# andrenarchy/krypy

Hardware: AMD Instinct MI355X
Metric: GMRES iterations/sec + SpMV HBM GB/s, n=10^7 5-pt Laplacian fp64 (higher is better)
Workload: dtype f64; 1 GPU; GMRES(100) restart cycles, 2-D 5-pt Laplacian 4000x2500 CSR (N=10000000, nnz=49987000), b=rng(0) normal, x0=0, tol=1e-8 (BASELINE.json configs[1]); n=10000000, ortho=mgs, restart=100, parallelism=1 GPU, ranks=1

## Files before the change

### krypy_amd/csrc/chain.h

```cpp
#pragma once
#include <type_traits>
#include "kernels.h"

namespace kh {

constexpr int CH_BS = 512;
constexpr int CH_GMAX = 512;

struct ChainArgs {
    int64_t n2;
    int64_t chunk2;
    const double* V;
    const double* B;
    int64_t ld;
    int64_t col0;
    int ncol;
    int sweeps;
    const double* w_in;
    const double* dg;
    double* vnext;
    double* pnext;
    double* hdev;
    int64_t hnext;
    unsigned long long* gran;
// ... 525 lines not shown
            int64_t c = row + a.offs.off[d];
            c = c < 0 ? 0 : (c > last ? last : c);
            xv[d] = xk[c];
        }
        double sx = 0.0, sy = 0.0;
#pragma unroll
        for (int d = 0; d < FND; ++d) {
            const double px = av[d].x * xv[d].x - av[d].y * xv[d].y;
            const double py = av[d].x * xv[d].y + av[d].y * xv[d].x;
            const bool on = (av[d].x != 0.0) || (av[d].y != 0.0);
            sx = on ? sx + px : sx;
            sy = on ? sy + py : sy;
        }
        put(r, sx, sy);
        if ((r & 1) == 1) asm volatile("" : "+v"(fb) : : "memory");
    }
}

template <int R2, int FND, int RIF, bool MASK, class Put>
__device__ __forceinline__ void chain_apply_banded_form(const ChainArgs& a, int64_t first, Put&& put) {
    const double* __restrict__ xk = a.xk;
    const int64_t last = a.n_last;
    int64_t fb = first;
#pragma unroll
    for (int r = 0; r < R2; ++r) {
        const int64_t i2 = fb + (int64_t)r * CH_BS;
        const int64_t row = 2 * i2;
        double2 av[FND];
        double x0[FND], x1[FND];
        const unsigned m = MASK ? dia_mask_load(a.dmask, i2) : 0u;
#pragma unroll
        for (int d = 0; d < FND; ++d) {
            const int64_t off = a.offs.off[d];
            av[d] = dia_slot<MASK>(a.dia, a.dia_ld, d, i2, m, MASK ? a.offs.cst[d] : 0.0);
            int64_t c0 = row + off, c1 = row + 1 + off;
            c0 = c0 < 0 ? 0 : (c0 > last ? last : c0);
            c1 = c1 < 0 ? 0 : (c1 > last ? last : c1);
            x0[d] = xk[c0];
            x1[d] = xk[c1];
        }
        double s0 = 0.0, s1 = 0.0;
#pragma unroll
        for (int d = 0; d < FND; ++d) {
            const double p0 = av[d].x * x0[d], p1 = av[d].y * x1[d];
            s0 = (av[d].x != 0.0) ? s0 + p0 : s0;
            s1 = (av[d].y != 0.0) ? s1 + p1 : s1;
        }
        put(r, s0, s1);
        if ((r & RIF) == RIF) asm volatile("" : "+v"(fb) : : "memory");
    }
}

template <int R2, int FND, int RIF = KH_RIF, class Put>
__device__ __forceinline__ void chain_apply_banded(const ChainArgs& a, int64_t first, Put&& put) {
    static_assert(FND <= KH_DIA_CMAX, "the mask form holds up to KH_DIA_CMAX diagonals");
    if (a.dmask != nullptr) chain_apply_banded_form<R2, FND, RIF, true>(a, first, put);
    else chain_apply_banded_form<R2, FND, RIF, false>(a, first, put);
}

template <int R2, bool MASKED, bool CPLX = false, int FND = 0, int WL = 0, bool ONEX = false, bool XR = false>
__global__ __launch_bounds__(CH_BS) void k_mgs_chain(ChainArgs a) {
    static_assert(FND == 0 || !MASKED, "the fused operator exists for the padded kernels");
    static_assert(!XR || (!CPLX && !ONEX), "the cross-rank stage exists for real vectors spread over the chip");
    constexpr int RW = R2 - WL;
    extern __shared__ __attribute__((aligned(16))) double2 wl[];
#define W_GET(r) (((r) < RW) ? w[((r) < RW) ? (r) : 0] : wl[((r) - RW) * CH_BS + tid])
#define W_PUT(r, val)                                   \
    do {                                                \
        if ((r) < RW) w[((r) < RW) ? (r) : 0] = (val);  \
        else wl[((r) - RW) * CH_BS + tid] = (val);      \
    } while (0)
    constexpr int PB = ChainShape<R2>::PB;
    constexpr int NB = ChainShape<R2>::NB;
    __shared__ double smd[4 * (CH_BS / 64)];
    __shared__ unsigned smu[2 * CH_GMAX];
    __shared__ int slead;
    const int tid = threadIdx.x;
    int G = gridDim.x;
    int bid = blockIdx.x;
    GridRole role;
    if constexpr (ONEX) {
        if (!onex_enter(a, &slead, bid, G, role)) return;
    } else {
        role = grid_role(a.xcc_leader, a.epoch0, &slead);
    }
    const int64_t first = (int64_t)bid * a.chunk2 + tid;
    const int64_t left = a.n2 - first;
    const int rem = (int)(left < 0 ? 0 : (left > a.chunk2 ? a.chunk2 : left));
#define CH_OK(r) (!MASKED || (r) * CH_BS < rem)
    double2 w[RW];
    double2 ring[2][PB];
    if constexpr (FND > 0 && CPLX) {
        chain_apply_banded_z<R2, FND>(a, first, [&](int r, double s0, double s1) { W_PUT(r, make_double2(s0, s1)); });
    } else if constexpr (FND > 0) {
        chain_apply_banded<R2, FND>(a, first, [&](int r, double s0, double s1) { W_PUT(r, make_double2(s0, s1)); });
    } else {
        const double2* __restrict__ win2 = reinterpret_cast<const double2*>(a.w_in) + first;
#pragma unroll
        for (int r = 0; r < R2; ++r) {
            const double2 v = win2[(int64_t)r * CH_BS];
            double2 t;
            t.x = CH_OK(r) ? v.x : 0.0;
            t.y = CH_OK(r) ? v.y : 0.0;
            W_PUT(r, t);
            if ((r + 1) % 8 == 0) CH_ISSUE_FENCE();
        }
    }
    if (a.presub) {
        const double hk = (a.h_km1_dev != nullptr) ? a.h_km1_dev[0] : a.h_km1;
        const double2* __restrict__ p2 = reinterpret_cast<const double2*>(a.bprev) + first;
#pragma unroll
        for (int r = 0; r < R2; ++r) {
            const double2 p = p2[(int64_t)r * CH_BS];
            double2 t = W_GET(r);
            t.x = CH_OK(r) ? t.x - hk * p.x : 0.0;
            t.y = CH_OK(r) ? t.y - hk * p.y : 0.0;
            W_PUT(r, t);
            if ((r + 1) % 8 == 0) CH_ISSUE_FENCE();
        }
    }
    unsigned epoch = a.epoch0;
    if (a.debug == 4 && tid == 0) __hip_atomic_store(a.err, 1, __ATOMIC_RELAXED, __HIP_MEMORY_SCOPE_AGENT);
    const int total = a.ncol * a.sweeps;
    {
        const double2* __restrict__ v2 = reinterpret_cast<const double2*>(a.V + a.col0 * a.ld) + first;
#pragma unroll
        for (int i = 0; i < PB; ++i) ring[0][i] = v2[(int64_t)i * CH_BS];
        CH_ISSUE_FENCE();
    }
    for (int t = 0; t < total; ++t) {
        const int64_t j = a.col0 + (t % a.ncol);
        const double2* __restrict__ v2 = reinterpret_cast<const double2*>(a.V + j * a.ld) + first;
        const double2* __restrict__ b2 = reinterpret_cast<const double2*>(a.B + j * a.ld) + first;
        double acc0 = 0.0, acc1 = 0.0;
        if (a.debug != 2)
#pragma unroll
        for (int b = 0; b < NB; ++b) {
            const double2* __restrict__ nx = (b + 1 < NB) ? v2 + (int64_t)(b + 1) * PB * CH_BS : b2;
#pragma unroll
            for (int i = 0; i < PB; ++i)
                ring[(b + 1) & 1][i] = (WL > 0 && b + 1 == NB) ? ld_nt2(nx + (int64_t)i * CH_BS) : nx[(int64_t)i * CH_BS];
            CH_ISSUE_FENCE();
#pragma unroll
            for (int i = 0; i < PB; ++i) {
                double2 v = ring[b & 1][i];
                if (MASKED && !CH_OK(b * PB + i)) v = make_double2(0.0, 0.0);
                const double2 wr = W_GET(b * PB + i);
                if (CPLX) {
                    acc0 = fma(v.x, wr.x, acc0);
                    acc0 = fma(v.y, wr.y, acc0);
                    acc1 = fma(v.x, wr.y, acc1);
                    acc1 = fma(-v.y, wr.x, acc1);
                } else {
                    acc0 = fma(v.x, wr.x, acc0);
                    acc1 = fma(v.y, wr.y, acc1);
                }
            }
        }
        double alpha, alpha_i = 0.0;
        if (CPLX) {
            alpha = acc0;
            alpha_i = acc1;
            if constexpr (ONEX) {
                double pv[2] = {alpha, alpha_i};
                onex_sum<2>(pv, epoch++, a.gran, G, bid, a.err, smd);
                alpha = pv[0];
                alpha_i = pv[1];
            } else {
                grid_sum2(alpha, alpha_i, epoch++, a.gran, G, a.err, smd, smu, role, a.xcc_res);
            }
            if (bid == 0 && tid == 0) {
                a.hdev[2 * j] = (t < a.ncol ? 0.0 : a.hdev[2 * j]) + alpha;
                a.hdev[2 * j + 1] = (t < a.ncol ? 0.0 : a.hdev[2 * j + 1]) + alpha_i;
            }
        } else {
            if constexpr (ONEX) {
                double pv[1] = {acc0 + acc1};
                onex_sum<1>(pv, epoch++, a.gran, G, bid, a.err, smd);
                alpha = pv[0];
            } else {
                const unsigned e_ = epoch++;
                alpha = (a.debug == 1) ? (acc0 + acc1) * 1e-30
                                       : grid_sum<XR>(acc0 + acc1, e_, a.gran, G, a.err, smd, smu, role, a.xcc_res, nullptr, &a.xr,
                                                      a.xr.epoch0 + (e_ - a.epoch0));
            }
            if (bid == 0 && tid == 0) a.hdev[j] = (t < a.ncol ? 0.0 : a.hdev[j]) + alpha;
        }
        if (a.debug == 4) alpha *= 0.5;
        const int64_t jn = a.col0 + ((t + 1) % a.ncol);
        const double2* __restrict__ vn = (t + 1 < total)
            ? reinterpret_cast<const double2*>(a.V + jn * a.ld) + first
            : reinterpret_cast<const double2*>(a.w_in) + first;
        if (a.debug != 2)
#pragma unroll
        for (int b = 0; b < NB; ++b) {
            const double2* __restrict__ nx = (b + 1 < NB) ? b2 + (int64_t)(b + 1) * PB * CH_BS : vn;
#pragma unroll
            for (int i = 0; i < PB; ++i)
                ring[(b + 1) & 1][i] = (WL > 0 && b + 1 < NB) ? ld_nt2(nx + (int64_t)i * CH_BS) : nx[(int64_t)i * CH_BS];
            CH_ISSUE_FENCE();
#pragma unroll
            for (int i = 0; i < PB; ++i) {
                const double2 p = ring[b & 1][i];
                const int r = b * PB + i;
                double2 wr = W_GET(r);
                if (CPLX) {
                    const double tr = alpha * p.x - alpha_i * p.y;
                    const double ti = alpha * p.y + alpha_i * p.x;
                    wr.x = CH_OK(r) ? wr.x - tr : 0.0;
                    wr.y = CH_OK(r) ? wr.y - ti : 0.0;
                } else {
                    wr.x = CH_OK(r) ? wr.x - alpha * p.x : 0.0;
                    wr.y = CH_OK(r) ? wr.y - alpha * p.y : 0.0;
                }
                W_PUT(r, wr);
            }
        }
    }
    double acc = 0.0;
    if (a.dg != nullptr) {
        const double2* __restrict__ d2 = reinterpret_cast<const double2*>(a.dg) + first;
#pragma unroll
        for (int r = 0; r < R2; ++r) {
            const double2 d = d2[(int64_t)r * CH_BS];
            const double2 wr = W_GET(r);
            acc = fma(wr.x, d.x * wr.x, acc);
            acc = fma(wr.y, d.y * wr.y, acc);
            if ((r + 1) % 8 == 0) CH_ISSUE_FENCE();
        }
    } else {
#pragma unroll
        for (int r = 0; r < R2; ++r) {
            const double2 wr = W_GET(r);
            acc = fma(wr.x, wr.x, acc);
            acc = fma(wr.y, wr.y, acc);
        }
    }
    double h2;
    if constexpr (ONEX) {
        double pv[1] = {acc};
        onex_sum<1>(pv, epoch++, a.gran, G, bid, a.err, smd);
        h2 = pv[0];
    } else {
        const unsigned e_ = epoch++;
        h2 = grid_sum<XR>(acc, e_, a.gran, G, a.err, smd, smu, role, a.xcc_res, nullptr, &a.xr, a.xr.epoch0 + (e_ - a.epoch0));
    }
    const double h = sqrt(fabs(h2));
    if (bid == 0 && tid == 0) a.hdev[a.hnext] = h;
    double2* __restrict__ vn2 = reinterpret_cast<double2*>(a.vnext) + first;
    if (a.dg != nullptr) {
        double2* __restrict__ pn2 = reinterpret_cast<double2*>(a.pnext) + first;
        const double2* __restrict__ d2 = reinterpret_cast<const double2*>(a.dg) + first;
#pragma unroll
        for (int r = 0; r < R2; ++r) {
            if (r * CH_BS < rem) {
                const double2 d = d2[(int64_t)r * CH_BS];
                const double2 wr = W_GET(r);
                double2 o, m;
                o.x = wr.x / h;
                o.y = wr.y / h;
                m.x = (d.x * wr.x) / h;
                m.y = (d.y * wr.y) / h;
                st_nt2(pn2 + (int64_t)r * CH_BS, o);
                st_nt2(vn2 + (int64_t)r * CH_BS, m);
            }
        }
    } else {
#pragma unroll
        for (int r = 0; r < R2; ++r) {
            if (r * CH_BS < rem) {
                const double2 wr = W_GET(r);
                double2 o;
                o.x = wr.x / h;
                o.y = wr.y / h;
                st_nt2(vn2 + (int64_t)r * CH_BS, o);
            }
        }
    }
    if (bid == 0 && a.hpin != nullptr) {
        __syncthreads();
        for (int i = tid; i < a.hcount; i += CH_BS)
            a.hpin[i] = __hip_atomic_load(a.hdev + i, __ATOMIC_RELAXED, __HIP_MEMORY_SCOPE_AGENT);
        if (tid == 0) *a.errpin = __hip_atomic_load(a.err, __ATOMIC_RELAXED, __HIP_MEMORY_SCOPE_AGENT);
        CH_SIGNAL_DONE(a);
    }
#undef W_PUT
#undef W_GET
#undef CH_OK
}

#ifndef KH_CH_REUSE_SKIP
#define KH_CH_REUSE_SKIP 0
#endif
#ifndef KH_CH_SKIP_LAST
#define KH_CH_SKIP_LAST 0
#endif
#ifndef KH_CH_LDS_EARLY
#define KH_CH_LDS_EARLY 0
#endif
template <int R2, bool CPLX = false>
struct ChainShapeLds {
    static constexpr int PB = ChainShape<R2>::PB;
    static constexpr int NB = R2 / PB;
    static constexpr int LB = NB >= 4 ? 3 : 1;
    static constexpr int NG = NB - LB - 1;
    static_assert((NB % 2) == 0 && NG >= 0 && (NG % 2) == 0, "ring parity must reset every phase");
    static constexpr int WL = (R2 == 40 && !CPLX) ? 4 : 0;
    static constexpr size_t LDS_BYTES = (size_t)(LB * PB + WL) * CH_BS * sizeof(double2);
};

template <int R2, bool MASKED, bool CPLX = false, int FND = 0, bool XR = false>
__global__ __launch_bounds__(CH_BS) void k_mgs_chain_lds(ChainArgs a) {
    static_assert(FND == 0 || !MASKED, "the fused operator exists for the padded kernels");
    static_assert(!XR || !CPLX, "the cross-rank stage exists for real vectors");
    constexpr int PB = ChainShapeLds<R2, CPLX>::PB;
    constexpr int NB = ChainShapeLds<R2, CPLX>::NB;
    constexpr int LB = ChainShapeLds<R2, CPLX>::LB;
    constexpr int NG = ChainShapeLds<R2, CPLX>::NG;
    constexpr int WL = ChainShapeLds<R2, CPLX>::WL;
    constexpr int RW = R2 - WL;
    extern __shared__ __attribute__((aligned(16))) double2 vlds[];
    double2* const wl = vlds + (size_t)LB * PB * CH_BS;
#define W_GET(r) (((r) < RW) ? w[((r) < RW) ? (r) : 0] : wl[((r) - RW) * CH_BS + tid])
#define W_PUT(r, val)                                   \
    do {                                                \
        if ((r) < RW) w[((r) < RW) ? (r) : 0] = (val);  \
        else wl[((r) - RW) * CH_BS + tid] = (val);      \
    } while (0)
    __shared__ double smd[4 * (CH_BS / 64)];
    __shared__ unsigned smu[2 * CH_GMAX];
    __shared__ int slead;
    const int tid = threadIdx.x;
    const int G = gridDim.x;
    const GridRole role = grid_role(a.xcc_leader, a.epoch0, &slead);
    const int64_t first = (int64_t)blockIdx.x * a.chunk2 + tid;
    const int64_t left = a.n2 - first;
    const int rem = (int)(left < 0 ? 0 : (left > a.chunk2 ? a.chunk2 : left));
#define CH_OK(r) (!MASKED || (r) * CH_BS < rem)
#define CH_LD(ptr, reuse) ((reuse) ? *(ptr) : ld_nt2(ptr))
    double2 w[RW];
    double2 ring[2][PB];
    if constexpr (FND > 0 && CPLX) {
        chain_apply_banded_z<R2, FND>(a, first, [&](int r, double s0, double s1) { W_PUT(r, make_double2(s0, s1)); });
    } else if constexpr (FND > 0) {
        chain_apply_banded<R2, FND>(a, first, [&](int r, double s0, double s1) { W_PUT(r, make_double2(s0, s1)); });
    } else {
        const double2* __restrict__ win2 = reinterpret_cast<const double2*>(a.w_in) + first;
#pragma unroll
        for (int r = 0; r < R2; ++r) {
            const double2 v = ld_nt2(win2 + (int64_t)r * CH_BS);
            double2 t;
            t.x = CH_OK(r) ? v.x : 0.0;
            t.y = CH_OK(r) ? v.y : 0.0;
            W_PUT(r, t);
            if ((r + 1) % 8 == 0) CH_ISSUE_FENCE();
        }
    }
    if (a.presub) {
        const double hk = (a.h_km1_dev != nullptr) ? a.h_km1_dev[0] : a.h_km1;
        const double2* __restrict__ p2 = reinterpret_cast<const double2*>(a.bprev) + first;
#pragma unroll
        for (int r = 0; r < R2; ++r) {
            const double2 p = p2[(int64_t)r * CH_BS];
            double2 t = W_GET(r);
            t.x = CH_OK(r) ? t.x - hk * p.x : 0.0;
            t.y = CH_OK(r) ? t.y - hk * p.y : 0.0;
            W_PUT(r, t);
            if ((r + 1) % 8 == 0) CH_ISSUE_FENCE();
        }
    }
    unsigned epoch = a.epoch0;
    if (a.debug == 4 && tid == 0) __hip_atomic_store(a.err, 1, __ATOMIC_RELAXED, __HIP_MEMORY_SCOPE_AGENT);
    const int total = a.ncol * a.sweeps;
    {
        const double2* __restrict__ v2 = reinterpret_cast<const double2*>(a.V + a.col0 * a.ld) + first;
#pragma unroll
        for (int i = 0; i < PB; ++i) ring[0][i] = CH_LD(v2 + (int64_t)i * CH_BS, false);
        CH_ISSUE_FENCE();
    }
#if defined(KH_CHAIN_TRACE) && KH_CHAIN_TRACE == 2
    unsigned long long tr_acc[9] = {0, 0, 0, 0, 0, 0, 0, 0, 0};
#endif
    for (int t = 0; t < total; ++t) {
        const int64_t j = a.col0 + (t % a.ncol);
        const double2* __restrict__ v2 = reinterpret_cast<const double2*>(a.V + j * a.ld) + first;
        const int64_t jn = a.col0 + ((t + 1) % a.ncol);
        const double2* __restrict__ vn = (t + 1 < total)
            ? reinterpret_cast<const double2*>(a.V + jn * a.ld) + first
            : reinterpret_cast<const double2*>(a.w_in) + first;
        double acc0 = 0.0, acc1 = 0.0;
        CH_STAMP(a, t, total, 0);
#pragma unroll
        for (int b = 0; b < NB; ++b) {
            const double2* __restrict__ nx = (b + 1 < NB) ? v2 + (int64_t)(b + 1) * PB * CH_BS
                                                            : (NG > 0 ? v2 + (int64_t)(NB - 2) * PB * CH_BS : vn);
#pragma unroll
            for (int i = 0; i < PB; ++i)
                ring[(b + 1) & 1][i] = CH_LD(nx + (int64_t)i * CH_BS, (b + 1 < NB) && (b + 1 >= LB + KH_CH_REUSE_SKIP) && (b + 1 <= NB - 2 - KH_CH_SKIP_LAST));
            CH_ISSUE_FENCE();
#pragma unroll
            for (int i = 0; i < PB; ++i) {
                double2 v = ring[b & 1][i];
                if (MASKED && !CH_OK(b * PB + i)) v = make_double2(0.0, 0.0);
                if (b < LB) vlds[(b * PB + i) * CH_BS + tid] = v;
                const double2 wr = W_GET(b * PB + i);
                if (CPLX) {
                    acc0 = fma(v.x, wr.x, acc0);
                    acc0 = fma(v.y, wr.y, acc0);
                    acc1 = fma(v.x, wr.y, acc1);
                    acc1 = fma(-v.y, wr.x, acc1);
                } else {
                    acc0 = fma(v.x, wr.x, acc0);
                    acc1 = fma(v.y, wr.y, acc1);
                }
            }
        }
        double alpha, alpha_i = 0.0;
        CH_STAMP(a, t, total, 1);
        if (CPLX) {
            alpha = acc0;
            alpha_i = acc1;
            grid_sum2(alpha, alpha_i, epoch++, a.gran, G, a.err, smd, smu, role, a.xcc_res);
            if (blockIdx.x == 0 && tid == 0) {
                a.hdev[2 * j] = (t < a.ncol ? 0.0 : a.hdev[2 * j]) + alpha;
                a.hdev[2 * j + 1] = (t < a.ncol ? 0.0 : a.hdev[2 * j + 1]) + alpha_i;
            }
        } else {
#if defined(KH_CHAIN_TRACE) && KH_CHAIN_TRACE == 2
            alpha = grid_sum(acc0 + acc1, epoch++, a.gran, G, a.err, smd, smu, role, a.xcc_res, tr_acc);
#elif defined(KH_CHAIN_TRACE)
            alpha = grid_sum(acc0 + acc1, epoch++, a.gran, G, a.err, smd, smu, role, a.xcc_res,
                             a.trace ? a.trace + (((size_t)blockIdx.x * total) + t) * 16 : nullptr);
#else
            const unsigned e_ = epoch++;
            alpha = (a.debug == 1) ? (acc0 + acc1) * 1e-30
                                   : grid_sum<XR>(acc0 + acc1, e_, a.gran, G, a.err, smd, smu, role, a.xcc_res, nullptr, &a.xr,
                                                  a.xr.epoch0 + (e_ - a.epoch0));
#endif
            if (blockIdx.x == 0 && tid == 0) a.hdev[j] = (t < a.ncol ? 0.0 : a.hdev[j]) + alpha;
        }
        if (a.debug == 4) alpha *= 0.5;
        CH_STAMP(a, t, total, 5);
#define CH_UPD(r, p)                                              \
    do {                                                          \
        double2 wr_ = W_GET(r);                                   \
        if (CPLX) {                                               \
            const double tr = alpha * (p).x - alpha_i * (p).y;    \
            const double ti = alpha * (p).y + alpha_i * (p).x;    \
            wr_.x = CH_OK(r) ? wr_.x - tr : 0.0;                  \
            wr_.y = CH_OK(r) ? wr_.y - ti : 0.0;                  \
        } else {                                                  \
            wr_.x = CH_OK(r) ? wr_.x - alpha * (p).x : 0.0;       \
            wr_.y = CH_OK(r) ? wr_.y - alpha * (p).y : 0.0;       \
        }                                                         \
        W_PUT(r, wr_);                                            \
    } while (0)
#pragma unroll
        for (int i = 0; i < PB; ++i) CH_UPD((NB - 1) * PB + i, ring[1][i]);
        constexpr bool EARLY = (KH_CH_LDS_EARLY != 0) && NG >= 2;
#pragma unroll
        for (int g = 0; g < NG; ++g) {
            const int b = NB - 2 - g;
            const double2* __restrict__ nx = (g + 1 < NG) ? v2 + (int64_t)(b - 1) * PB * CH_BS : vn;
#pragma unroll
            for (int i = 0; i < PB; ++i) ring[(g + 1) & 1][i] = CH_LD(nx + (int64_t)i * CH_BS, false);
            CH_ISSUE_FENCE();
            if (EARLY && g == 1) {
#pragma unroll
                for (int bb = LB - 1; bb >= 0; --bb) {
#pragma unroll
                    for (int i = 0; i < PB; ++i) {
                        const double2 p = vlds[(bb * PB + i) * CH_BS + tid];
                        CH_UPD(bb * PB + i, p);
                    }
                    CH_ISSUE_FENCE();
                }
            }
#pragma unroll
            for (int i = 0; i < PB; ++i) CH_UPD(b * PB + i, ring[g & 1][i]);
        }
        CH_STAMP(a, t, total, 6);
        if (!EARLY) {
#pragma unroll
            for (int b = LB - 1; b >= 0; --b) {
                CH_ISSUE_FENCE();
#pragma unroll
                for (int i = 0; i < PB; ++i) {
                    const double2 p = vlds[(b * PB + i) * CH_BS + tid];
                    CH_UPD(b * PB + i, p);
                }
            }
        }
#undef CH_UPD
        CH_STAMP(a, t, total, 7);
    }
#if defined(KH_CHAIN_TRACE) && KH_CHAIN_TRACE == 2
    if (a.trace != nullptr && (tid == 0 || tid == CH_BS - 64)) {
#pragma unroll
        for (int i = 0; i < 8; ++i) a.trace[((size_t)blockIdx.x * 2 + (tid ? 1 : 0)) * 8 + i] = tr_acc[i];
    }
#endif
    double acc = 0.0;
    if (a.dg != nullptr) {
        const double2* __restrict__ d2 = reinterpret_cast<const double2*>(a.dg) + first;
#pragma unroll
        for (int r = 0; r < R2; ++r) {
            const double2 d = d2[(int64_t)r * CH_BS];
            const double2 wr = W_GET(r);
            acc = fma(wr.x, d.x * wr.x, acc);
            acc = fma(wr.y, d.y * wr.y, acc);
            if ((r + 1) % 8 == 0) CH_ISSUE_FENCE();
        }
    } else {
#pragma unroll
        for (int r = 0; r < R2; ++r) {
            const double2 wr = W_GET(r);
            acc = fma(wr.x, wr.x, acc);
            acc = fma(wr.y, wr.y, acc);
        }
    }
    const unsigned en_ = epoch++;
    const double h2 = grid_sum<XR>(acc, en_, a.gran, G, a.err, smd, smu, role, a.xcc_res, nullptr, &a.xr, a.xr.epoch0 + (en_ - a.epoch0));
    const double h = sqrt(fabs(h2));
    if (blockIdx.x == 0 && tid == 0) a.hdev[a.hnext] = h;
    double2* __restrict__ vn2 = reinterpret_cast<double2*>(a.vnext) + first;
    if (a.dg != nullptr) {
        double2* __restrict__ pn2 = reinterpret_cast<double2*>(a.pnext) + first;
        const double2* __restrict__ d2 = reinterpret_cast<const double2*>(a.dg) + first;
#pragma unroll
        for (int r = 0; r < R2; ++r) {
            if (r * CH_BS < rem) {
                const double2 d = d2[(int64_t)r * CH_BS];
                const double2 wr = W_GET(r);
                double2 o, m;
                o.x = wr.x / h;
                o.y = wr.y / h;
                m.x = (d.x * wr.x) / h;
                m.y = (d.y * wr.y) / h;
                st_nt2(pn2 + (int64_t)r * CH_BS, o);
                st_nt2(vn2 + (int64_t)r * CH_BS, m);
            }
        }
    } else {
#pragma unroll
        for (int r = 0; r < R2; ++r) {
            if (r * CH_BS < rem) {
                const double2 wr = W_GET(r);
                double2 o;
                o.x = wr.x / h;
                o.y = wr.y / h;
                st_nt2(vn2 + (int64_t)r * CH_BS, o);
            }
        }
    }
    if (blockIdx.x == 0 && a.hpin != nullptr) {
        __syncthreads();
        for (int i = tid; i < a.hcount; i += CH_BS)
            a.hpin[i] = __hip_atomic_load(a.hdev + i, __ATOMIC_RELAXED, __HIP_MEMORY_SCOPE_AGENT);
        if (tid == 0) *a.errpin = __hip_atomic_load(a.err, __ATOMIC_RELAXED, __HIP_MEMORY_SCOPE_AGENT);
        CH_SIGNAL_DONE(a);
    }
#undef W_PUT
#undef W_GET
#undef CH_LD
#undef CH_OK
}

template <int R2>
struct ChainShapePf {
    static constexpr int PB = ChainShape<R2>::PB;
    static constexpr int NB = R2 / PB;
    static constexpr int LB = (NB - 2 < 3) ? NB - 2 : 3;
    static constexpr int NG = NB - 2 - LB;
    static_assert((NB % 2) == 0 && NB >= 2 && LB >= 0 && NG >= 0 && NG <= LB, "shape");
    static constexpr int ROW_BYTES = CH_BS * (int)sizeof(double2);
    static constexpr int STATIC_LDS = 2 * (CH_BS / 64) * 8 + 2 * CH_GMAX * 4 + 256;
    static constexpr int SPARE = (160 * 1024 - STATIC_LDS - LB * PB * ROW_BYTES) / ROW_BYTES;
#ifndef KH_PF_SP_CAP
#define KH_PF_SP_CAP 64
#endif
    static constexpr int SP0 = SPARE < PB ? SPARE : PB;
    static constexpr int SP = SP0 < KH_PF_SP_CAP ? SP0 : KH_PF_SP_CAP;
    static_assert(SP0 >= 1, "at least one spare row");
    static constexpr size_t LDS_BYTES = (size_t)(LB * PB + SP) * ROW_BYTES;
};

typedef __attribute__((address_space(3))) double2 ch_lds_double2;

__device__ __forceinline__ void ch_dma16(const double2* gsrc, unsigned lds_dst) {
    unsigned keep;
    asm volatile("s_mov_b32 %0, m0\n\ts_mov_b32 m0, %2\n\ts_nop 0\n\tglobal_load_lds_dwordx4 %1, off\n\ts_mov_b32 m0, %0"
                 : "=&s"(keep)
                 : "v"(gsrc), "s"(lds_dst)
                 : "memory");
}

template <int R2, bool MASKED, bool CPLX = false, int FND = 0, bool ONEX = false>
__global__ __launch_bounds__(CH_BS) void k_mgs_chain_pf(ChainArgs a) {
    static_assert(FND == 0 || (!MASKED && !CPLX), "the fused operator exists for the padded real kernel");
    constexpr int PB = ChainShapePf<R2>::PB;
    constexpr int NB = ChainShapePf<R2>::NB;
    constexpr int LB = ChainShapePf<R2>::LB;
    constexpr int NG = ChainShapePf<R2>::NG;
    constexpr int SP = ChainShapePf<R2>::SP;
    extern __shared__ __attribute__((aligned(16))) double2 vlds[];
    double2* const vsp = vlds + (size_t)LB * PB * CH_BS;
    __shared__ double smd[4 * (CH_BS / 64)];
    __shared__ unsigned smu[2 * CH_GMAX];
    __shared__ int slead;
    const int tid = threadIdx.x;
    int G = gridDim.x;
    int bid = blockIdx.x;
    GridRole role;
    if constexpr (ONEX) {
        if (!onex_enter(a, &slead, bid, G, role)) return;
    } else {
        role = grid_role(a.xcc_leader, a.epoch0, &slead);
    }
    const int64_t first = (int64_t)bid * a.chunk2 + tid;
    const int64_t left = a.n2 - first;
    const int rem = (int)(left < 0 ? 0 : (left > a.chunk2 ? a.chunk2 : left));
    const unsigned lds_wave = (unsigned)(size_t)((ch_lds_double2*)vlds) +
                              (unsigned)__builtin_amdgcn_readfirstlane((tid >> 6) * 64 * (int)sizeof(double2));
#define CH_OK(r) (!MASKED || (r) * CH_BS < rem)
#define CH_LD(ptr, reuse) ((reuse) ? *(ptr) : ld_nt2(ptr))
    double2 w[R2];
    double2 ring[2][PB];
    if constexpr (FND > 0) {
        chain_apply_banded<R2, FND>(a, first, [&](int r, double s0, double s1) { w[r] = make_double2(s0, s1); });
    } else {
        const double2* __restrict__ win2 = reinterpret_cast<const double2*>(a.w_in) + first;
#pragma unroll
        for (int r = 0; r < R2; ++r) {
            const double2 v = ld_nt2(win2 + (int64_t)r * CH_BS);
            w[r].x = CH_OK(r) ? v.x : 0.0;
            w[r].y = CH_OK(r) ? v.y : 0.0;
            if ((r + 1) % 8 == 0) CH_ISSUE_FENCE();
        }
    }
    if (a.presub) {
        const double hk = (a.h_km1_dev != nullptr) ? a.h_km1_dev[0] : a.h_km1;
        const double2* __restrict__ p2 = reinterpret_cast<const double2*>(a.bprev) + first;
#pragma unroll
        for (int r = 0; r < R2; ++r) {
            const double2 p = p2[(int64_t)r * CH_BS];
            w[r].x = CH_OK(r) ? w[r].x - hk * p.x : 0.0;
            w[r].y = CH_OK(r) ? w[r].y - hk * p.y : 0.0;
            if ((r + 1) % 8 == 0) CH_ISSUE_FENCE();
        }
    }
    unsigned epoch = a.epoch0;
    if (a.debug == 4 && tid == 0) __hip_atomic_store(a.err, 1, __ATOMIC_RELAXED, __HIP_MEMORY_SCOPE_AGENT);
    const int total = a.ncol * a.sweeps;
#define CH_REUSE(b) ((b) >= LB && (b) < LB + NG)
    {
        const double2* __restrict__ v2 = reinterpret_cast<const double2*>(a.V + a.col0 * a.ld) + first;
#pragma unroll
        for (int i = 0; i < SP; ++i)
            ch_dma16(v2 + (int64_t)i * CH_BS, lds_wave + (unsigned)(((LB * PB + i) * CH_BS) * sizeof(double2)));
#pragma unroll
        for (int i = SP; i < PB; ++i) ring[0][i] = CH_LD(v2 + (int64_t)i * CH_BS, CH_REUSE(0));
        CH_ISSUE_FENCE();
        if (NB > 1) {
#pragma unroll
            for (int i = 0; i < PB; ++i) ring[1][i] = CH_LD(v2 + (int64_t)(PB + i) * CH_BS, CH_REUSE(1));
            CH_ISSUE_FENCE();
        }
    }
    for (int t = 0; t < total; ++t) {
        const int64_t j = a.col0 + (t % a.ncol);
        const double2* __restrict__ v2 = reinterpret_cast<const double2*>(a.V + j * a.ld) + first;
        const int64_t jn = a.col0 + ((t + 1) % a.ncol);
        const double2* __restrict__ vn = (t + 1 < total)
            ? reinterpret_cast<const double2*>(a.V + jn * a.ld) + first
            : reinterpret_cast<const double2*>(a.w_in) + first;
        double acc0 = 0.0, acc1 = 0.0;
        asm volatile("s_waitcnt vmcnt(%0)" ::"n"(2 * PB - SP) : "memory");
#pragma unroll
        for (int b = 0; b < NB; ++b) {
#pragma unroll
            for (int i = 0; i < PB; ++i) {
                double2 v = (b == 0 && i < SP) ? vsp[i * CH_BS + tid] : ring[b & 1][i];
                if (MASKED && !CH_OK(b * PB + i)) v = make_double2(0.0, 0.0);
                if (NB == 2 && b == 0 && i < SP) ring[0][i] = v;
                if (b < LB) vlds[(b * PB + i) * CH_BS + tid] = v;
                if (CPLX) {
                    acc0 = fma(v.x, w[b * PB + i].x, acc0);
                    acc0 = fma(v.y, w[b * PB + i].y, acc0);
                    acc1 = fma(v.x, w[b * PB + i].y, acc1);
                    acc1 = fma(-v.y, w[b * PB + i].x, acc1);
                } else {
                    acc0 = fma(v.x, w[b * PB + i].x, acc0);
                    acc1 = fma(v.y, w[b * PB + i].y, acc1);
                }
            }
            if (b + 2 < NB) {
                CH_ISSUE_FENCE();
#pragma unroll
                for (int i = 0; i < PB; ++i)
                    ring[b & 1][i] = CH_LD(v2 + (int64_t)((b + 2) * PB + i) * CH_BS, CH_REUSE(b + 2));
                CH_ISSUE_FENCE();
            }
        }
        asm volatile("s_waitcnt lgkmcnt(0)" ::: "memory");
#pragma unroll
        for (int i = 0; i < SP; ++i)
            ch_dma16(vn + (int64_t)i * CH_BS, lds_wave + (unsigned)(((LB * PB + i) * CH_BS) * sizeof(double2)));
        double alpha, alpha_i = 0.0;
        if (CPLX) {
            alpha = acc0;
            alpha_i = acc1;
            if constexpr (ONEX) {
                double pv[2] = {alpha, alpha_i};
                onex_sum<2>(pv, epoch++, a.gran, G, bid, a.err, smd);
                alpha = pv[0];
                alpha_i = pv[1];
            } else {
                grid_sum2(alpha, alpha_i, epoch++, a.gran, G, a.err, smd, smu, role, a.xcc_res);
            }
            if (bid == 0 && tid == 0) {
                a.hdev[2 * j] = (t < a.ncol ? 0.0 : a.hdev[2 * j]) + alpha;
                a.hdev[2 * j + 1] = (t < a.ncol ? 0.0 : a.hdev[2 * j + 1]) + alpha_i;
            }
        } else {
            if constexpr (ONEX) {
                double pv[1] = {acc0 + acc1};
                onex_sum<1>(pv, epoch++, a.gran, G, bid, a.err, smd);
                alpha = pv[0];
            } else {
                alpha = (a.debug == 1) ? (acc0 + acc1) * 1e-30
                                       : grid_sum(acc0 + acc1, epoch++, a.gran, G, a.err, smd, smu, role, a.xcc_res);
            }
            if (bid == 0 && tid == 0) a.hdev[j] = (t < a.ncol ? 0.0 : a.hdev[j]) + alpha;
        }
        if (a.debug == 4) alpha *= 0.5;
#define CH_UPD(r, p)                                              \
    do {                                                          \
        if (CPLX) {                                               \
            const double tr = alpha * (p).x - alpha_i * (p).y;    \
            const double ti = alpha * (p).y + alpha_i * (p).x;    \
            w[r].x = CH_OK(r) ? w[r].x - tr : 0.0;                \
            w[r].y = CH_OK(r) ? w[r].y - ti : 0.0;                \
        } else {                                                  \
            w[r].x = CH_OK(r) ? w[r].x - alpha * (p).x : 0.0;     \
            w[r].y = CH_OK(r) ? w[r].y - alpha * (p).y : 0.0;     \
        }                                                         \
    } while (0)
#pragma unroll
        for (int b = 0; b < LB; ++b) {
            CH_ISSUE_FENCE();
#pragma unroll
            for (int i = 0; i < PB; ++i) {
                const double2 p = vlds[(b * PB + i) * CH_BS + tid];
                CH_UPD(b * PB + i, p);
            }
        }
        if constexpr (NG > 0) {
            asm volatile("s_waitcnt lgkmcnt(0)" ::: "memory");
#pragma unroll
            for (int g = 0; g < NG; ++g)
#pragma unroll
                for (int i = 0; i < PB; ++i)
                    ch_dma16(v2 + (int64_t)((LB + g) * PB + i) * CH_BS,
                             lds_wave + (unsigned)(((g * PB + i) * CH_BS) * sizeof(double2)));
        }
        if (NB > 1) {
#pragma unroll
            for (int i = 0; i < PB; ++i) CH_UPD((NB - 2) * PB + i, ring[0][i]);
            CH_ISSUE_FENCE();
#pragma unroll
            for (int i = SP; i < PB; ++i) ring[0][i] = CH_LD(vn + (int64_t)i * CH_BS, CH_REUSE(0));
            CH_ISSUE_FENCE();
#pragma unroll
            for (int i = 0; i < PB; ++i) CH_UPD((NB - 1) * PB + i, ring[1][i]);
            CH_ISSUE_FENCE();
#pragma unroll
            for (int i = 0; i < PB; ++i) ring[1][i] = CH_LD(vn + (int64_t)(PB + i) * CH_BS, CH_REUSE(1));
            CH_ISSUE_FENCE();
        }
        if constexpr (NG > 0) {
            asm volatile("s_waitcnt vmcnt(%0)" ::"n"(2 * PB - SP) : "memory");
#pragma unroll
            for (int g = 0; g < NG; ++g) {
                CH_ISSUE_FENCE();
#pragma unroll
                for (int i = 0; i < PB; ++i) {
                    const double2 p = vlds[(g * PB + i) * CH_BS + tid];
                    CH_UPD((LB + g) * PB + i, p);
                }
            }
        }
#undef CH_UPD
    }
    double acc = 0.0;
#pragma unroll
    for (int r = 0; r < R2; ++r) {
        acc = fma(w[r].x, w[r].x, acc);
        acc = fma(w[r].y, w[r].y, acc);
    }
    double h2;
    if constexpr (ONEX) {
        double pv[1] = {acc};
        onex_sum<1>(pv, epoch++, a.gran, G, bid, a.err, smd);
        h2 = pv[0];
    } else {
        h2 = grid_sum(acc, epoch++, a.gran, G, a.err, smd, smu, role, a.xcc_res);
    }
    const double h = sqrt(fabs(h2));
    if (bid == 0 && tid == 0) a.hdev[a.hnext] = h;
    double2* __restrict__ vn2 = reinterpret_cast<double2*>(a.vnext) + first;
#pragma unroll
    for (int r = 0; r < R2; ++r) {
        if (r * CH_BS < rem) {
            double2 o;
            o.x = w[r].x / h;
            o.y = w[r].y / h;
            st_nt2(vn2 + (int64_t)r * CH_BS, o);
        }
    }
    if (bid == 0 && a.hpin != nullptr) {
        __syncthreads();
        for (int i = tid; i < a.hcount; i += CH_BS)
            a.hpin[i] = __hip_atomic_load(a.hdev + i, __ATOMIC_RELAXED, __HIP_MEMORY_SCOPE_AGENT);
        if (tid == 0) *a.errpin = __hip_atomic_load(a.err, __ATOMIC_RELAXED, __HIP_MEMORY_SCOPE_AGENT);
        CH_SIGNAL_DONE(a);
    }
#undef CH_REUSE
#undef CH_LD
#undef CH_OK
}

template <int R2, int LA, bool MASKED, int FND = 0, bool ONEX = false, bool DMASK = false>
__global__ __launch_bounds__(ONEX ? CH_BS + 64 : CH_BS) void k_mgs_chain_small(ChainArgs a) {
    static_assert(FND == 0 || !MASKED, "the fused operator exists for padded blocks");
    static_assert(FND > 0 || !DMASK, "the mask form is a form of the fused operator");
    constexpr int NS = LA + 1;
    __shared__ double smd[4 * (CH_BS / 64)];
    __shared__ unsigned smu[2 * CH_GMAX];
    __shared__ int slead;
    const int tid = threadIdx.x;
    int G = gridDim.x;
    int bid = blockIdx.x;
    GridRole role;
    if constexpr (ONEX) {
        if (!onex_enter(a, &slead, bid, G, role)) return;
    } else {
        role = grid_role(a.xcc_leader, a.epoch0, &slead);
    }
    unsigned epoch = a.epoch0;
    const int total = a.ncol * a.sweeps;
    if constexpr (ONEX) {
        if (tid >= CH_BS) {
            const bool writer = bid == 0 && tid == CH_BS;
            for (int t = 0; t < total; ++t) {
                const double alpha = onex_sum_comm(epoch++, a.gran, G, bid, a.err, smd);
                const int64_t j = a.col0 + (t % a.ncol);
                if (writer) a.hdev[j] = (t < a.ncol ? 0.0 : a.hdev[j]) + alpha;
            }
            const double h2 = onex_sum_comm(epoch++, a.gran, G, bid, a.err, smd);
            if (writer) a.hdev[a.hnext] = sqrt(fabs(h2));
            if (bid == 0 && a.hpin != nullptr) {
                __syncthreads();
                if (a.donepin != nullptr) __syncthreads();
            }
            return;
        }
// ... 391 lines not shown
```

Baseline: 1160 iterations/s.

## Repack LDS rows in MGS chain kernel: park 19 basis rows, keep w in registers

For the R2=40 real shape, the LDS budget is reorganized. The four spilled rows of w are now held in registers after the prologue, and the freed LDS space parks more basis-vector rows (19 instead of 12). That count is not a multiple of the batch size, so the batch loops gain per-row split predicates. Parking more rows means fewer basis-vector rows are re-read from HBM in the update sweep. The cost is higher register pressure from holding all of w in registers, which may reduce occupancy or cause spills.

Result: faster. 1213 iterations/s (median of 6 runs) (+4.5%).

```diff
diff --git a/krypy_amd/csrc/chain.h b/krypy_amd/csrc/chain.h
--- a/krypy_amd/csrc/chain.h
+++ b/krypy_amd/csrc/chain.h
@@ -851,11 +851,14 @@
 struct ChainShapeLds {
     static constexpr int PB = ChainShape<R2>::PB;
     static constexpr int NB = R2 / PB;
-    static constexpr int LB = NB >= 4 ? 3 : 1;
-    static constexpr int NG = NB - LB - 1;
+    static constexpr int WL = (R2 == 40 && !CPLX) ? 4 : 0;
+    static constexpr int LROWS = (R2 == 40 && !CPLX) ? 19 : (NB >= 4 ? 3 : 1) * PB;
+    static constexpr int NG = NB - 1 - LROWS / PB;
     static_assert((NB % 2) == 0 && NG >= 0 && (NG % 2) == 0, "ring parity must reset every phase");
-    static constexpr int WL = (R2 == 40 && !CPLX) ? 4 : 0;
-    static constexpr size_t LDS_BYTES = (size_t)(LB * PB + WL) * CH_BS * sizeof(double2);
+    static_assert(WL <= LROWS && LROWS <= R2 - PB, "the prologue's rows of w borrow parked rows; the last batch stays in the ring");
+    static constexpr size_t LDS_BYTES = (size_t)LROWS * CH_BS * sizeof(double2);
+    static constexpr size_t STATIC_LDS = 4 * (CH_BS / 64) * sizeof(double) + 2 * CH_GMAX * sizeof(unsigned) + sizeof(int);
+    static_assert(LDS_BYTES + STATIC_LDS <= 160 * 1024, "a CU has 160 KB of LDS");
 };
 
 template <int R2, bool MASKED, bool CPLX = false, int FND = 0, bool XR = false>
@@ -864,18 +867,21 @@
     static_assert(!XR || !CPLX, "the cross-rank stage exists for real vectors");
     constexpr int PB = ChainShapeLds<R2, CPLX>::PB;
     constexpr int NB = ChainShapeLds<R2, CPLX>::NB;
-    constexpr int LB = ChainShapeLds<R2, CPLX>::LB;
+    constexpr int LROWS = ChainShapeLds<R2, CPLX>::LROWS;
+    constexpr int LBC = (LROWS + PB - 1) / PB;
+    constexpr bool SPLIT = (LROWS % PB) != 0;
     constexpr int NG = ChainShapeLds<R2, CPLX>::NG;
-    constexpr int WL = ChainShapeLds<R2, CPLX>::WL;
+    constexpr int WL = FND > 0 ? ChainShapeLds<R2, CPLX>::WL : 0;
     constexpr int RW = R2 - WL;
     extern __shared__ __attribute__((aligned(16))) double2 vlds[];
-    double2* const wl = vlds + (size_t)LB * PB * CH_BS;
-#define W_GET(r) (((r) < RW) ? w[((r) < RW) ? (r) : 0] : wl[((r) - RW) * CH_BS + tid])
-#define W_PUT(r, val)                                   \
-    do {                                                \
-        if ((r) < RW) w[((r) < RW) ? (r) : 0] = (val);  \
-        else wl[((r) - RW) * CH_BS + tid] = (val);      \
+#define W_GET_N(r, NR) (((r) < (NR)) ? w[((r) < (NR)) ? (r) : 0] : vlds[((r) - (NR)) * CH_BS + tid])
+#define W_PUT_N(r, val, NR)                                 \
+    do {                                                    \
+        if ((r) < (NR)) w[((r) < (NR)) ? (r) : 0] = (val);  \
+        else vlds[((r) - (NR)) * CH_BS + tid] = (val);      \
     } while (0)
+#define W_GET(r) W_GET_N(r, RW)
+#define W_PUT(r, val) W_PUT_N(r, val, RW)
     __shared__ double smd[4 * (CH_BS / 64)];
     __shared__ unsigned smu[2 * CH_GMAX];
     __shared__ int slead;
@@ -887,7 +893,7 @@
     const int rem = (int)(left < 0 ? 0 : (left > a.chunk2 ? a.chunk2 : left));
 #define CH_OK(r) (!MASKED || (r) * CH_BS < rem)
 #define CH_LD(ptr, reuse) ((reuse) ? *(ptr) : ld_nt2(ptr))
-    double2 w[RW];
+    double2 w[R2];
     double2 ring[2][PB];
     if constexpr (FND > 0 && CPLX) {
         chain_apply_banded_z<R2, FND>(a, first, [&](int r, double s0, double s1) { W_PUT(r, make_double2(s0, s1)); });
@@ -918,6 +924,15 @@
             if ((r + 1) % 8 == 0) CH_ISSUE_FENCE();
         }
     }
+    if constexpr (WL > 0) {
+#pragma unroll
+        for (int r = RW; r < R2; ++r) w[r] = vlds[(r - RW) * CH_BS + tid];
+        CH_ISSUE_FENCE();
+    }
+#undef W_PUT
+#undef W_GET
+#define W_GET(r) W_GET_N(r, R2)
+#define W_PUT(r, val) W_PUT_N(r, val, R2)
     unsigned epoch = a.epoch0;
     if (a.debug == 4 && tid == 0) __hip_atomic_store(a.err, 1, __ATOMIC_RELAXED, __HIP_MEMORY_SCOPE_AGENT);
     const int total = a.ncol * a.sweeps;
@@ -944,14 +959,17 @@
             const double2* __restrict__ nx = (b + 1 < NB) ? v2 + (int64_t)(b + 1) * PB * CH_BS
                                                             : (NG > 0 ? v2 + (int64_t)(NB - 2) * PB * CH_BS : vn);
 #pragma unroll
-            for (int i = 0; i < PB; ++i)
-                ring[(b + 1) & 1][i] = CH_LD(nx + (int64_t)i * CH_BS, (b + 1 < NB) && (b + 1 >= LB + KH_CH_REUSE_SKIP) && (b + 1 <= NB - 2 - KH_CH_SKIP_LAST));
+            for (int i = 0; i < PB; ++i) {
+                if (!SPLIT || b + 1 < NB || NG == 0 || (NB - 2) * PB + i >= LROWS)
+                    ring[(b + 1) & 1][i] = CH_LD(nx + (int64_t)i * CH_BS, (b + 1 < NB) && (!SPLIT || (b + 1) * PB + i >= LROWS) &&
+                                                                              (b + 1 >= LROWS / PB + KH_CH_REUSE_SKIP) && (b + 1 <= NB - 2 - KH_CH_SKIP_LAST));
+            }
             CH_ISSUE_FENCE();
 #pragma unroll
             for (int i = 0; i < PB; ++i) {
                 double2 v = ring[b & 1][i];
                 if (MASKED && !CH_OK(b * PB + i)) v = make_double2(0.0, 0.0);
-                if (b < LB) vlds[(b * PB + i) * CH_BS + tid] = v;
+                if (SPLIT ? (b * PB + i < LROWS) : (b < LBC)) vlds[(b * PB + i) * CH_BS + tid] = v;
                 const double2 wr = W_GET(b * PB + i);
                 if (CPLX) {
                     acc0 = fma(v.x, wr.x, acc0);
@@ -1012,31 +1030,39 @@
             const int b = NB - 2 - g;
             const double2* __restrict__ nx = (g + 1 < NG) ? v2 + (int64_t)(b - 1) * PB * CH_BS : vn;
 #pragma unroll
-            for (int i = 0; i < PB; ++i) ring[(g + 1) & 1][i] = CH_LD(nx + (int64_t)i * CH_BS, false);
+            for (int i = 0; i < PB; ++i) {
+                if (!SPLIT || g + 1 == NG || (b - 1) * PB + i >= LROWS) ring[(g + 1) & 1][i] = CH_LD(nx + (int64_t)i * CH_BS, false);
+            }
             CH_ISSUE_FENCE();
             if (EARLY && g == 1) {
 #pragma unroll
-                for (int bb = LB - 1; bb >= 0; --bb) {
+                for (int bb = LBC - 1; bb >= 0; --bb) {
 #pragma unroll
                     for (int i = 0; i < PB; ++i) {
-                        const double2 p = vlds[(bb * PB + i) * CH_BS + tid];
-                        CH_UPD(bb * PB + i, p);
+                        if (!SPLIT || bb * PB + i < LROWS) {
+                            const double2 p = vlds[(bb * PB + i) * CH_BS + tid];
+                            CH_UPD(bb * PB + i, p);
+                        }
                     }
                     CH_ISSUE_FENCE();
                 }
             }
 #pragma unroll
-            for (int i = 0; i < PB; ++i) CH_UPD(b * PB + i, ring[g & 1][i]);
+            for (int i = 0; i < PB; ++i) {
+                if (!SPLIT || b * PB + i >= LROWS) CH_UPD(b * PB + i, ring[g & 1][i]);
+            }
         }
         CH_STAMP(a, t, total, 6);
         if (!EARLY) {
 #pragma unroll
-            for (int b = LB - 1; b >= 0; --b) {
+            for (int b = LBC - 1; b >= 0; --b) {
                 CH_ISSUE_FENCE();
 #pragma unroll
                 for (int i = 0; i < PB; ++i) {
-                    const double2 p = vlds[(b * PB + i) * CH_BS + tid];
-                    CH_UPD(b * PB + i, p);
+                    if (!SPLIT || b * PB + i < LROWS) {
+                        const double2 p = vlds[(b * PB + i) * CH_BS + tid];
+                        CH_UPD(b * PB + i, p);
+                    }
                 }
             }
         }
@@ -1111,6 +1137,8 @@
     }
 #undef W_PUT
 #undef W_GET
+#undef W_PUT_N
+#undef W_GET_N
 #undef CH_LD
 #undef CH_OK
 }
```
